# AntoinePassemiers/Oriana

Measured on NVIDIA B200. Metric: cavi_matrix_entries_per_sec, higher is better.
Workload: dtype tf32 operands / f32 accumulate (f32 state, f64 ELBO sums)

## Files before the change

include/oriana_b200.h:

```cpp
#ifndef ORIANA_B200_H
#define ORIANA_B200_H

#include <stddef.h>
#include <stdint.h>

#ifdef __cplusplus
extern "C" {
#endif

#define ORI_OK 0
#define ORI_EINVAL (-1)
#define ORI_ECUDA (-2)
#define ORI_ENODEV (-3)
#define ORI_EUNSUPPORTED (-4)

#define ORI_F_DROPOUT 1u
#define ORI_F_QUIRK 2u
#define ORI_F_ELBO 4u
#define ORI_F_NO_TENSOR 8u
#define ORI_F_SPARSE 16u
#define ORI_F_DEVICE_ITER 32u

#define ORI_F_PRECISE 64u
#define ORI_F_FIXED_CHAIN 128u
// ... 109 lines not shown
int ori_zigap_compute_Z_q_expectations_host(float* DZ_hat_i, float* DZ_hat_j, float* DZ_exp_logsum_hat,
                                            const float* log_U_hat, const float* log_V_hat,
                                            const float* D_hat, const float* X,
                                            int64_t n, int64_t p, int64_t K, int quirk);
int ori_gap_compute_Z_q_expectations_host(float* Z_hat_i, float* Z_hat_j,
                                          const float* log_U_hat, const float* log_V_hat,
                                          const float* X, int64_t n, int64_t p, int64_t K);
int ori_zigap_compute_Z_q_expectations_ctx(ori_ctx_t* ctx, float* DZ_hat_i, float* DZ_hat_j, float* DZ_exp_logsum_hat,
                                           const float* log_U_hat, const float* log_V_hat,
                                           const float* D_hat, const float* X,
                                           int64_t n, int64_t p, int64_t K, int quirk);
int ori_gap_compute_Z_q_expectations_ctx(ori_ctx_t* ctx, float* Z_hat_i, float* Z_hat_j,
                                         const float* log_U_hat, const float* log_V_hat,
                                         const float* X, int64_t n, int64_t p, int64_t K);

int ori_synth_counts_f32(float* X, int64_t ldx, int64_t row0, int64_t n_rows, int32_t p, int32_t K,
                         uint64_t seed, float zero_level, int nb, float* Ustar, float* Vstar, float* pi,
                         void* stream);

int ori_widen_counts_f32(const void* src, int elem_bytes, int64_t lds, float* dst, int64_t ldd,
                         int64_t rows, int32_t p, void* stream);

int ori_expand_bitmap_counts_f32(const uint32_t* bitmap, int64_t words_per_row, const uint8_t* nz,
                                 const int64_t* rowoff, int64_t base, float* dst, int64_t ldd, int64_t rows,
                                 int32_t p, void* stream);

int ori_scatter_counts_f32(float* X, int64_t ldx, int64_t row0, int64_t rows, int32_t p, const int32_t* row,
                           const int32_t* col, const float* val, int64_t count, void* stream);

#ifdef __cplusplus
// ... 4 lines not shown
```

oriana_b200/_lib.py:

```python
import ctypes as C
import os

_HERE = os.path.dirname(os.path.abspath(__file__))
LIB_PATH = os.environ.get('ORIANA_B200_LIB') or os.path.join(_HERE, 'lib', 'liboriana_b200.so')

ORI_F_DROPOUT, ORI_F_QUIRK, ORI_F_ELBO, ORI_F_NO_TENSOR, ORI_F_SPARSE, ORI_F_DEVICE_ITER, ORI_F_PRECISE = 1, 2, 4, 8, 16, 32, 64
ORI_F_FIXED_CHAIN = 128
ORI_F_DETERMINISTIC = 256
ORI_M_STEP, ORI_M_INIT, ORI_M_INIT_KEEP, ORI_M_FINALIZE, ORI_M_REFRESH = 0, 1, 2, 3, 4
R64_NSLOTS = 8
SCAL_SLOTS = 16

_fp = C.POINTER(C.c_float)
_dp = C.POINTER(C.c_double)


class OriProblem(C.Structure):
    _fields_ = [
        ('n_rows', C.c_int64), ('n_total', C.c_int64), ('ldx', C.c_int64),
        ('p', C.c_int32), ('K', C.c_int32), ('KP', C.c_int32), ('flags', C.c_uint32),
        ('iter', C.c_int32), ('trace_cap', C.c_int32),
        ('X', C.c_void_p),
        ('a1', C.c_void_p), ('a2', C.c_void_p),
        ('U_hat', C.c_void_p * 2), ('eU', C.c_void_p * 2),
# ... 37 lines not shown
    'ori_row_sums_f32': ([C.c_void_p, C.c_int64, C.c_int64, C.c_int32, C.c_void_p, C.c_void_p], C.c_int),
    'ori_column_sums_f64': ([C.c_void_p, C.c_int64, C.c_int64, C.c_int32, C.c_void_p, C.c_void_p], C.c_int),
    'ori_deviance_sums': ([_PP, C.c_int, C.c_void_p, C.c_void_p, C.c_void_p, C.c_void_p, C.c_void_p], C.c_int),
    'ori_zigap_compute_Z_q_expectations_host': ([C.c_void_p] * 7 + [C.c_int64] * 3 + [C.c_int], C.c_int),
    'ori_gap_compute_Z_q_expectations_host': ([C.c_void_p] * 5 + [C.c_int64] * 3, C.c_int),
    'ori_ctx_create': ([C.POINTER(C.c_void_p), C.c_int64], C.c_int),
    'ori_ctx_destroy': ([C.c_void_p], C.c_int),
    'ori_ctx_stats': ([C.c_void_p] + [C.POINTER(C.c_uint64)] * 4, C.c_int),
    'ori_zigap_compute_Z_q_expectations_ctx': ([C.c_void_p] * 8 + [C.c_int64] * 3 + [C.c_int], C.c_int),
    'ori_gap_compute_Z_q_expectations_ctx': ([C.c_void_p] * 6 + [C.c_int64] * 3, C.c_int),
    'ori_widen_counts_f32': ([C.c_void_p, C.c_int, C.c_int64, C.c_void_p, C.c_int64, C.c_int64, C.c_int32, C.c_void_p], C.c_int),
    'ori_expand_bitmap_counts_f32': ([C.c_void_p, C.c_int64, C.c_void_p, C.c_void_p, C.c_int64, C.c_void_p, C.c_int64, C.c_int64,
                                      C.c_int32, C.c_void_p], C.c_int),
    'ori_scatter_counts_f32': ([C.c_void_p, C.c_int64, C.c_int64, C.c_int64, C.c_int32, C.c_void_p, C.c_void_p, C.c_void_p,
                                C.c_int64, C.c_void_p], C.c_int),
    'ori_synth_counts_f32': ([C.c_void_p, C.c_int64, C.c_int64, C.c_int64, C.c_int32, C.c_int32, C.c_uint64,
                              C.c_float, C.c_int, C.c_void_p, C.c_void_p, C.c_void_p, C.c_void_p], C.c_int),
}

_lib = None


class OrianaB200Error(RuntimeError):
    pass


def exported_symbols():
    return sorted(_SIGNATURES)


# ... 39 lines not shown
```

oriana_b200/csrc/kernels_tc.cu:

```cuda
#include <cstring>
#include "common.cuh"
#include "tc_ptx.cuh"

namespace ori {
using namespace tc;

constexpr int TC_OWN = 128;
constexpr int NEW = 8;
constexpr int TC_THREADS = 64 + 32 * NEW;
constexpr int NCTA = 2;

template <int KP, bool PRECISE = false, bool DEVI = false>
struct Cfg {
    static_assert(KP == 32 || KP == 64, "tensor path: KP is 32 or 64");
    static_assert(!PRECISE || KP == 32, "the fp32-grade plan exists for KP = 32");
    static constexpr int SW = PRECISE ? 32 : 2048 / KP;
    static constexpr int NS = 2;
    static constexpr int KB = KP / 32;
    static constexpr int KST = 3, TST = 3, XST = 4;
    static constexpr int NTA = PRECISE ? 4 : 2;
    static constexpr uint32_t K_BLK = (SW / NCTA) * 128;
    static constexpr uint32_t K_ARR = KB * K_BLK;
    static constexpr uint32_t K_STAGE = 4 * K_ARR;
    static constexpr uint32_t T_CHUNK = (KP / NCTA) * 128;
// ... 55 lines not shown
    asm volatile("cp.async.bulk.shared::cluster.global.mbarrier::complete_tx::bytes [%0], [%1], %2, [%3];"
                 ::"r"(smem_u32(dst)), "l"(src), "r"(bytes), "r"(smem_u32(bar)) : "memory");
}
__device__ __forceinline__ uint32_t tf32_bias(float x) { return __float_as_uint(x) + 0x1000u; }

__device__ __forceinline__ float4 lds128(uint32_t a) {
    float4 v;
    asm volatile("ld.shared.v4.f32 {%0, %1, %2, %3}, [%4];" : "=f"(v.x), "=f"(v.y), "=f"(v.z), "=f"(v.w) : "r"(a));
    return v;
}
__device__ __forceinline__ float lds32(uint32_t a) {
    float v;
    asm volatile("ld.shared.f32 %0, [%1];" : "=f"(v) : "r"(a));
    return v;
}
__device__ __forceinline__ float sel_nz_a(float x, float a, float b) {
    float d;
    asm("{\n\t.reg .pred q;\n\tsetp.neu.f32 q, %1, 0f00000000;\n\tselp.f32 %0, %2, %3, q;\n\t}" : "=f"(d) : "f"(x), "f"(a), "f"(b));
    return d;
}
__device__ __forceinline__ float sel_nz_b(float x, float a, float b) {
    float d;
    asm("{\n\t.reg .pred q;\n\t.reg .f32 t;\n\tabs.f32 t, %1;\n\tsetp.gtu.f32 q, t, 0f00000000;\n\tselp.f32 %0, %2, %3, q;\n\t}"
        : "=f"(d) : "f"(x), "f"(a), "f"(b));
    return d;
}
__device__ __forceinline__ float is_zero_f(float x) {
    float d;
    asm("set.eq.f32.f32 %0, %1, 0f00000000;" : "=f"(d) : "f"(x));
    return d;
// ... 20 lines not shown
        }
    }
    __device__ __forceinline__ void init(const TcArgs& a, int ncta_, int rank_) {
        ncta = ncta_; rank = rank_;
        item = blockIdx.x / ncta; stride = gridDim.x / ncta;
        load(a);
    }
    __device__ __forceinline__ bool valid(const TcArgs& a) const { return item < a.n_items; }
    __device__ __forceinline__ bool first() const { return t == t_begin; }
    __device__ __forceinline__ bool last() const { return t == t_end - 1; }
    __device__ __forceinline__ void next(const TcArgs& a) {
        if (++t >= t_end) { item += stride; load(a); }
    }
};

template <bool GENES, bool DROPOUT, bool ELBO, int KP, bool PRECISE, bool DEVI = false, bool UFL = false, bool DET = false>
__global__ void __launch_bounds__(TC_THREADS, 1)
k_tc_pass(const __grid_constant__ TcMaps maps, const TcArgs a)
{
    using C = Cfg<KP, PRECISE, DEVI>;
    static_assert(!DEVI || (!GENES && DROPOUT && !ELBO && !PRECISE), "deviance pass: row orientation, two contractions");
    constexpr int SW = C::SW, NS = C::NS;
    constexpr uint32_t TM_UV = C::TM_UV;
    constexpr int KST = C::KST, TST = C::TST, XST = C::XST;
    constexpr uint32_t K_STAGE = C::K_STAGE, T_STAGE = C::T_STAGE, X_STAGE = C::X_STAGE, LP_STAGE = C::LP_STAGE;
    constexpr uint32_t OFF_K = C::OFF_K, OFF_T = C::OFF_T, OFF_X = C::OFF_X, OFF_LP = C::OFF_LP, OFF_BAR = C::OFF_BAR;
    constexpr uint32_t TM_STAGE = C::TM_STAGE, TM_ACC = C::TM_ACC, TM_A = C::TM_A, TM_COLS = C::TM_COLS;
    constexpr int B_KFULL = C::B_KFULL, B_KEMPTY = C::B_KEMPTY, B_TFULL = C::B_TFULL, B_TEMPTY = C::B_TEMPTY,
                  B_XFULL = C::B_XFULL, B_XEMPTY = C::B_XEMPTY, B_SREADY = C::B_SREADY, B_PREADY = C::B_PREADY,
                  B_ACC_READY = C::B_ACC_READY, B_ACC_FREE = C::B_ACC_FREE, B_A_READY = C::B_A_READY, NBARS = C::NBARS;
    constexpr int CW = SW / 2;
    constexpr int G = CW / 16;
    constexpr int NQ = DROPOUT ? 4 : 2;
    constexpr int NT = DROPOUT ? 2 : 1;
    const int rank = (int)cluster_ctarank();

// ... 65 lines not shown
                        for (int kb = 0; kb < C::KB; ++kb) {
                            uint8_t* dst = st + q * C::K_ARR + kb * C::K_BLK;
                            const int row = (int)(q * a.sw_pad + sw0 + (SW / NCTA) * rank);
                            tma_load_2d_pair(dst, &maps.swK, bar, 32 * kb, row, L2_EVICT_LAST);
                        }
                }
                __syncwarp();
            }
            {
                const uint32_t s = nk % XST;
                mbar_wait(&bars[B_XEMPTY + s], ((nk / XST) & 1) ^ 1, 11);
                if (elect_one()) {
                    uint8_t* st = smem + OFF_X + s * X_STAGE;
                    uint64_t* bar = &bars[B_XFULL + s];
                    const int sw0 = ik.t * SW;
                    mbar_expect_tx(bar, X_STAGE + ((!GENES && DROPOUT) ? LP_STAGE : 0));
                    if (DEVI) bulk_load(smem + OFF_LP + s * LP_STAGE, a.devlp + (long long)ik.t * (8 * SW), LP_STAGE, bar);
                    if (!GENES) {
#pragma unroll
                        for (int c = 0; c < SW / 32; ++c)
                            tma_load_2d_hint(st + c * (TC_OWN * 128), &maps.X, bar, sw0 + 32 * c, ik.own0, L2_EVICT_FIRST);
                        if (DROPOUT && !DEVI) {
                            bulk_load(smem + OFF_LP + s * LP_STAGE, a.lp2w + sw0, SW * 4, bar);
                            bulk_load(smem + OFF_LP + s * LP_STAGE + SW * 4, a.flw + sw0, SW * 4, bar);
                            bulk_load(smem + OFF_LP + s * LP_STAGE + SW * 8, a.cw + sw0, SW * 4, bar);
                        }
                    } else {
#pragma unroll
                        for (int c = 0; c < 4; ++c)
                            tma_load_2d_hint(st + c * (SW * 128), &maps.X, bar, ik.own0 + 32 * c, sw0, L2_EVICT_FIRST);
                    }
                }
                __syncwarp();
            }
            if (nk > 0) load_T();
            ++nk; ik.next(a);
        }
        if (nk > 0) load_T();
    } else if (warp == 1 || false) {
        if (rank == 0) {
            constexpr uint32_t idescS = make_idesc_tf32(TC_OWN * NCTA, SW, false, false);
// ... 130 lines not shown
                        plo[e] = pack_bf16x2(__uint_as_float(wlo[2 * e]), __uint_as_float(wlo[2 * e + 1]));
                    }
                    tmem_st8(tlane + TM_A + (2 * slice + 1) * KP + 8 * c16, phi);
                    tmem_st8(tlane + TM_A + (2 * slice + 1) * KP + KP / 2 + 8 * c16, plo);
                }
            }
            tmem_wait_st();
            tc_fence_before();
            __syncwarp();
            if (lane == 0) mbar_arrive_cluster(&bars[B_A_READY], 0);
        };

        uint32_t xoff[8];
#pragma unroll
        for (int k = 0; k < 8; ++k) xoff[k] = (uint32_t)(quarter * (SW * 128) + ((((lane >> 2) ^ k)) << 4) + (lane & 3) * 4);

        TileIter ti;
        ti.init(a, NCTA, rank);
        uint32_t it = 0;
        int li = 0;
        if (ti.valid(a)) a_load_store(ti.own0);
        while (ti.valid(a)) {
            const long long own_idx = (long long)ti.own0 + lrow;
            const bool own_ok = own_idx < a.own_total;
            const int next_item = ti.item + ti.stride;
            const bool has_next = next_item < a.n_items;
            const int next_own0 = ((next_item % a.n_own_units) * NCTA + rank) * TC_OWN;
            float lp2j = 0.f, flj = 0.f, cj = 0.f, ulim = 127.f;
            if (GENES && DROPOUT) {
                lp2j = a.lp2w[own_idx]; flj = a.flw[own_idx];
// ... 1 lines not shown
                ulim = fminf(127.f, 127.f + lp2j);
            }
            const float lp2f = fminf(lp2j, 3.0e38f);
            float thr_o = 0.f, den_lim = 0.f;
            if constexpr (UFL) {
                thr_o = own_ok ? a.thr_own[own_idx] : 0.f;
                den_lim = thr_o * __ldg(a.thr_sw_max);
                den_lim = den_lim == den_lim ? fminf(den_lim, 3.0e38f) : 0.f;
            }
            const bool slow_item = DROPOUT && (GENES ? (__any_sync(0xffffffffu, flj != 0.f || lp2j == -INFINITY) != 0) : any_floor);
            float cs = 0.f;
            float xl_s = 0.f, xl_c = 0.f, ent_s = 0.f, ent_c = 0.f;
            const int t_end = ti.t_end;
            uint32_t dr[2][16], ur[2][16];
            float x[2][16];
            struct Tile { uint32_t xs_addr, lp_addr, tden, s, xs; int valid; bool slow; long long sw0; };
            auto tile_of = [&](uint32_t it_, int t_) {
                Tile c;
                c.s = it_ % NS; c.xs = it_ % XST;
                c.xs_addr = sbase + OFF_X + c.xs * X_STAGE;
                c.lp_addr = sbase + OFF_LP + c.xs * LP_STAGE;
                c.valid = (int)min((long long)SW, a.sw_total - (long long)t_ * SW);
                c.sw0 = (long long)t_ * SW;
                c.slow = slow_item || (GENES && c.valid != SW);
                c.tden = tlane + c.s * TM_STAGE;
                return c;
            };
            auto wait_tile = [&](uint32_t it_) {
                const uint32_t s = it_ % NS, sph = (it_ / NS) & 1, xs = it_ % XST, xph = (it_ / XST) & 1;
                mbar_wait2(&bars[B_XFULL + xs], xph, &bars[B_SREADY + s], sph, 30);
// ... 12 lines not shown
                    w[e] = __float_as_uint(h0); w[e + 1] = __float_as_uint(h1);
                    ph[e >> 1] = pack_bf16x2(h0, h1);
                    pl[e >> 1] = pack_bf16x2(v0 - h0, v1 - h1);
                }
            };
            auto load_x = [&](const Tile& c, int g, int b) {
                const int c0 = colbase + g * 16;
                if (!GENES) {
                    const uint32_t base = c.xs_addr + (c0 >> 5) * (TC_OWN * 128) + lrow * 128;
                    const int cb = (c0 & 31) >> 2;
#pragma unroll
                    for (int q = 0; q < 4; ++q) {
                        const float4 v = lds128(base + (((cb + q) ^ (lrow & 7)) << 4));
                        x[b][4 * q] = v.x; x[b][4 * q + 1] = v.y; x[b][4 * q + 2] = v.z; x[b][4 * q + 3] = v.w;
                    }
                } else {
#pragma unroll
                    for (int e = 0; e < 16; ++e) {
                        const int i = c0 + e;
                        x[b][e] = lds32(c.xs_addr + xoff[i & 7] + i * 128);
                    }
                }
            };
            auto slow_group = [&](const Tile& c, int g, int b, float& t_xl, float& t_ent) {
                const int c0 = colbase + g * 16;
                tmem_ld16(c.tden + c0, dr[b]);
                if (DROPOUT) tmem_ld16(c.tden + TM_UV + c0, ur[b]);
                tmem_wait_ld();
#pragma unroll
                for (int e = 0; e < 16; ++e) {
                    const float den = __uint_as_float(dr[b][e]);
                    const float xe = x[b][e];
                    const bool nz = xe != 0.f;
                    float xr = xe;
                    if constexpr (UFL)
                        if (den_lim > 0.f && nz && (c0 + e) < c.valid && den < thr_o * __ldg(a.thr_sw + c.sw0 + c0 + e)) xr = 0.f;
                    const float dg = den > 0.f ? den : 1.f;
                    float tt = dg, e2 = 0.f, D = 1.f;
                    if (DROPOUT) {
                        const float lp2 = GENES ? lp2j : lds32(c.lp_addr + 4 * (c0 + e));
                        const float fl = GENES ? flj : lds32(c.lp_addr + SW * 4 + 4 * (c0 + e));
                        e2 = fminf(__uint_as_float(ur[b][e]) - lp2, 127.f);
                        tt = nz ? dg : 1.f + ex2_approx(e2);
                        const float r = rcp_approx(tt);
                        D = fmaxf(nz ? 1.f : r, fl);
                        dr[b][e] = PRECISE ? __float_as_uint(xr * r) : tf32_bias(xr * r);
                        ur[b][e] = PRECISE ? __float_as_uint(D) : tf32_bias(D);
// ... 13 lines not shown
            };
            auto fast_group = [&](const Tile& c, int g, int b, float& g_cs, float& g_xl, float& g_ent) -> float {
                const int c0 = colbase + g * 16;
                float cc[16];
                if (DROPOUT && !GENES) {
#pragma unroll
                    for (int q = 0; q < 4; ++q) {
                        const float4 v = lds128(c.lp_addr + SW * 8 + 4 * (c0 + 4 * q));
                        cc[4 * q] = v.x; cc[4 * q + 1] = v.y; cc[4 * q + 2] = v.z; cc[4 * q + 3] = v.w;
                    }
                }
                float dmin = 1.f;
#pragma unroll
                for (int e = 0; e < 16; ++e) {
                    const float den = __uint_as_float(dr[b][e]);
                    const float xe = x[b][e];
                    dmin = fminf(dmin, den);
                    float tt = den, uvp = 0.f;
                    if (DROPOUT) {
                        uvp = __uint_as_float(ur[b][e]);
                        if (GENES && ELBO) uvp = fminf(uvp, ulim);
                        const float tz = fmaf(ex2_approx(uvp), GENES ? cj : cc[e], 1.f);
                        tt = sel_nz_a(xe, den, tz);
                    }
                    const float r = rcp_approx(tt);
                    dr[b][e] = PRECISE ? __float_as_uint(xe * r) : tf32_bias(xe * r);
                    float D = 1.f;
                    if (DROPOUT) {
                        D = sel_nz_b(xe, 1.f, r);
                        ur[b][e] = PRECISE ? __float_as_uint(D) : tf32_bias(D);
                    }
// ... 477 lines not shown
                                            P->n_rows, w.np, P->KP);
    return check_launch("k_tc_prep(rows, logsum)");
}

static void tc_partition(TcArgs& a, bool genes, int units, int sw, bool precise, bool fixed_chain) {
    int tpc = (precise ? ORI_TC_CHUNK_PRECISE : (genes ? ORI_TC_CHUNK : 2 * ORI_TC_CHUNK)) / sw;
    if (tpc < 1) tpc = 1;
    if (tpc > a.n_sw_tiles) tpc = a.n_sw_tiles;
    const int min_tpc = (128 / sw) > 1 ? 128 / sw : 1;
    while (!fixed_chain && (long long)a.n_own_units * cdiv(a.n_sw_tiles, tpc) < units / 2 && tpc > min_tpc) tpc = (tpc + 1) / 2;
    a.tiles_per_chunk = tpc;
    a.n_chunks = cdiv(a.n_sw_tiles, a.tiles_per_chunk);
    a.n_items = a.n_own_units * a.n_chunks;
}

template <bool GENES, bool D, bool E, int KP, bool PRECISE, bool DEVI, bool UFL, bool DET>
static int launch_tc_variant(const TcMaps& maps, const TcArgs& a, int grid, cudaStream_t st) {
    auto kern = k_tc_pass<GENES, D, E, KP, PRECISE, DEVI, UFL, DET>;
    constexpr uint32_t smem = Cfg<KP, PRECISE, DEVI>::SMEM_BYTES;
    static bool attr_done = false;
    if (!attr_done) {
        cudaError_t e_ = cudaFuncSetAttribute(kern, cudaFuncAttributeMaxDynamicSharedMemorySize, smem);
        if (e_ != cudaSuccess) return set_error(ORI_ECUDA, "cudaFuncSetAttribute: %s", cudaGetErrorString(e_));
        attr_done = true;
    }
    cudaLaunchConfig_t cfg = {};
    cfg.gridDim = dim3(grid); cfg.blockDim = dim3(TC_THREADS); cfg.dynamicSmemBytes = smem; cfg.stream = st;
    cudaLaunchAttribute attr[1];
    attr[0].id = cudaLaunchAttributeClusterDimension;
    attr[0].val.clusterDim.x = NCTA; attr[0].val.clusterDim.y = 1; attr[0].val.clusterDim.z = 1;
    cfg.attrs = attr; cfg.numAttrs = 1;
    cudaError_t e_ = cudaLaunchKernelEx(&cfg, kern, maps, a);
    if (e_ != cudaSuccess) return set_error(ORI_ECUDA, "cudaLaunchKernelEx(k_tc_pass): %s", cudaGetErrorString(e_));
    return ORI_OK;
}

template <bool GENES, int KP, bool PRECISE, bool UFL, bool DET>
static int launch_tc_flags(bool drop, bool elbo, const TcMaps& maps, const TcArgs& a, int grid, cudaStream_t st) {
    if (drop && elbo) return launch_tc_variant<GENES, true, true, KP, PRECISE, false, UFL, DET>(maps, a, grid, st);
    if (drop) return launch_tc_variant<GENES, true, false, KP, PRECISE, false, UFL, DET>(maps, a, grid, st);
    if (elbo) return launch_tc_variant<GENES, false, true, KP, PRECISE, false, UFL, DET>(maps, a, grid, st);
    return launch_tc_variant<GENES, false, false, KP, PRECISE, false, UFL, DET>(maps, a, grid, st);
}

template <bool GENES, int KP, bool PRECISE>
static int launch_tc_pass_p(const ori_problem_t* P, int gen_old, cudaStream_t st, bool logsum = false) {
    using C = Cfg<KP, PRECISE>;
    const TcWs w = tc_carve(P);
    const bool sparse = P->flags & ORI_F_SPARSE;
    const bool drop = (P->flags & ORI_F_DROPOUT) && !logsum, elbo = (P->flags & ORI_F_ELBO) && !logsum;
    constexpr int SW = C::SW;
    TcMaps maps;
    TcArgs a;
    bool ok;
    if (!GENES) {
        ok = make_tmap_f32(&maps.swK, w.geneK, 4 * w.pp, KP, KP, 32, SW / NCTA) &&
             make_tmap_f32(&maps.swT, w.geneT, C::NTA * KP, w.pp, w.pp, 32, KP / NCTA) &&
             make_tmap_f32(&maps.X, P->X, P->n_rows, P->p, P->ldx, 32, TC_OWN);
        a.own_total = P->n_rows; a.sw_total = P->p; a.sw_pad = w.pp;
        a.own_e = P->eU[gen_old]; a.own_E = P->U_hat[gen_old];
        a.acc1 = P->Zi; a.acc2 = P->a2s;
    } else {
        ok = make_tmap_f32(&maps.swK, w.rowK, 4 * w.np, KP, KP, 32, SW / NCTA) &&
             make_tmap_f32(&maps.swT, w.rowT, C::NTA * KP, w.np, w.np, 32, KP / NCTA) &&
             make_tmap_f32(&maps.X, P->X, P->n_rows, P->p, P->ldx, 32, SW);
        a.own_total = P->p; a.sw_total = P->n_rows; a.sw_pad = w.np;
        a.own_e = sparse ? P->eVd : P->eV; a.own_E = sparse ? P->Vh_old : P->V_hat;
        a.acc1 = P->red32 + (logsum ? 2ll * P->p * KP : 0ll); a.acc2 = P->red32 + (long long)P->p * KP;
    }
    if (!ok) return set_error(ORI_ECUDA, "cuTensorMapEncodeTiled failed");
    a.lp2w = w.lp2w; a.flw = w.flw; a.cw = w.cw; a.any_floor = w.flags;
    const bool ufl = P->thrU && P->thrV;
    const float* thr_rows = ufl ? P->thrU + (long long)gen_old * P->n_rows : nullptr;
    a.thr_own = ufl ? (GENES ? P->thrV : thr_rows) : nullptr;
    a.thr_sw = ufl ? (GENES ? thr_rows : P->thrV) : nullptr;
    a.thr_sw_max = ufl ? reinterpret_cast<const float*>(w.flags + (GENES ? 2 : 1)) : nullptr;
    a.colsum = P->red64; a.part64 = P->red64 + P->p + 2 * P->KP;
    a.n_own_tiles = cdiv(a.own_total, TC_OWN);
    a.n_own_units = cdiv(a.n_own_tiles, NCTA);
    a.n_sw_tiles = cdiv(a.sw_total, SW);
// ... 8 lines not shown
        a.colsum2 = P->det_ws + (long long)DET_FU_BLOCKS * DET_FU_SLOTS;
        a.item_part = a.colsum2 + pad128(P->p);
        if (GENES && drop) {
            const cudaError_t e2 = cudaMemsetAsync(a.colsum2, 0, sizeof(double) * (size_t)P->p, st);
            if (e2 != cudaSuccess) return set_error(ORI_ECUDA, "cudaMemsetAsync(colsum2): %s", cudaGetErrorString(e2));
        }
        a.tickets = reinterpret_cast<int*>(a.item_part + det_max_items(P->n_rows, P->p) * DET_ITEM_SLOTS);
        cudaError_t e_ = cudaMemsetAsync(a.tickets, 0, sizeof(int) * (size_t)(a.n_own_tiles + 2), st);
        if (e_ != cudaSuccess) return set_error(ORI_ECUDA, "cudaMemsetAsync(tickets): %s", cudaGetErrorString(e_));
        if (!(GENES && elbo)) a.item_part = nullptr;
        else {
            e_ = cudaMemsetAsync(a.item_part, 0, sizeof(double) * (size_t)a.n_items * DET_ITEM_SLOTS, st);
            if (e_ != cudaSuccess) return set_error(ORI_ECUDA, "cudaMemsetAsync(item_part): %s", cudaGetErrorString(e_));
        }
    }
    const int rc = det ? launch_tc_flags<GENES, KP, PRECISE, false, true>(drop, elbo, maps, a, grid, st)
                 : ufl ? launch_tc_flags<GENES, KP, PRECISE, true, false>(drop, elbo, maps, a, grid, st)
                       : launch_tc_flags<GENES, KP, PRECISE, false, false>(drop, elbo, maps, a, grid, st);
    if (rc != ORI_OK) return rc;
    int extra = 0;
    if (det && GENES && drop) { k_det_add<<<cdiv(P->p, 256), 256, 0, st>>>(P->red64, a.colsum2, P->p); ++extra; }
    if (a.item_part) {
        double* part = P->red64 + P->p + 2 * P->KP;
        k_det_sum_items<<<1, 1024, 0, st>>>(a.item_part, (long long)a.n_items * (DET_ITEM_SLOTS / 2), part + R64_XLOGDEN, part + R64_ENT);
        ++extra;
    }
    if (extra) return check_launch("k_tc_pass + deterministic sums", 1 + extra);
    return check_launch(GENES ? "k_tc_pass(genes)" : "k_tc_pass(rows)");
}

template <bool GENES>
static int launch_tc_pass(const ori_problem_t* P, int gen_old, cudaStream_t st, bool logsum = false) {
    if (P->flags & ORI_F_PRECISE) return launch_tc_pass_p<GENES, 32, true>(P, gen_old, st, logsum);
// ... 37 lines not shown
    while ((long long)a.n_own_units * cdiv(a.n_sw_tiles, a.tiles_per_chunk) < 2LL * units && a.tiles_per_chunk > 4)
        a.tiles_per_chunk = (a.tiles_per_chunk + 1) / 2;
    a.n_chunks = cdiv(a.n_sw_tiles, a.tiles_per_chunk);
    a.n_items = a.n_own_units * a.n_chunks;
    const int grid = NCTA * (a.n_items < units ? a.n_items : units);
    const int rc = launch_tc_variant<false, true, false, KP, false, true, false, false>(maps, a, grid, st);
    if (rc != ORI_OK) return rc;
    return check_launch("k_tc_pass(deviance)");
}

int launch_deviance_tc(const ori_problem_t* P, int g, const double* pi, const double* cmean, long long* out_int, cudaStream_t st) {
    if (P->KP == 64) return launch_deviance_tc_kp<64>(P, g, pi, cmean, out_int, st);
    return launch_deviance_tc_kp<32>(P, g, pi, cmean, out_int, st);
}

int launch_pass_rows_tc(const ori_problem_t* P, int gen_old, cudaStream_t st) { return launch_tc_pass<false>(P, gen_old, st); }
int launch_pass_genes_tc(const ori_problem_t* P, int gen_old, cudaStream_t st) { return launch_tc_pass<true>(P, gen_old, st); }
int launch_pass_genes_logsum_tc(const ori_problem_t* P, int gen_old, cudaStream_t st) { return launch_tc_pass<true>(P, gen_old, st, true); }

}
```

oriana_b200/csrc/synth.cu:

```cuda
#include "common.cuh"

namespace ori {

struct Philox {
    uint32_t k0, k1;
    __device__ Philox(uint64_t seed) : k0((uint32_t)seed), k1((uint32_t)(seed >> 32)) {}
    __device__ uint4 operator()(uint32_t c0, uint32_t c1, uint32_t c2, uint32_t c3) const {
        uint32_t a = k0, b = k1;
#pragma unroll
        for (int r = 0; r < 10; ++r) {
            const uint32_t h0 = __umulhi(0xD2511F53u, c0), l0 = 0xD2511F53u * c0;
            const uint32_t h1 = __umulhi(0xCD9E8D57u, c2), l1 = 0xCD9E8D57u * c2;
            c0 = h1 ^ c1 ^ a; c1 = l1; c2 = h0 ^ c3 ^ b; c3 = l0;
            a += 0x9E3779B9u; b += 0xBB67AE85u;
        }
        return make_uint4(c0, c1, c2, c3);
    }
};

__device__ __forceinline__ float u01(uint32_t x) { return ((float)(x >> 8) + 0.5f) * (1.0f / 16777216.0f); }

__global__ void k_synth_factor(float* __restrict__ out, long long rows, int K, long long row0, uint64_t seed, uint32_t tag) {
    const long long idx = (long long)blockIdx.x * blockDim.x + threadIdx.x;
    if (idx >= rows * K) return;
// ... 180 lines not shown
    if (e >= count) return;
    const long long r = (long long)row[e] - row0;
    const int c = col[e];
    if (r >= 0 && r < rows && c >= 0 && c < p) X[r * ldx + c] = val[e];
}

extern "C" int ori_scatter_counts_f32(float* X, int64_t ldx, int64_t row0, int64_t rows, int32_t p, const int32_t* row,
                                      const int32_t* col, const float* val, int64_t count, void* stream)
{
    if (!X || ldx < p || p <= 0 || rows < 0 || count < 0 || (count && (!row || !col || !val)))
        return set_error(ORI_EINVAL, "ori_scatter_counts_f32: bad argument");
    if (count == 0 || rows == 0) return ORI_OK;
    k_scatter_counts<<<cdiv(count, 256), 256, 0, (cudaStream_t)stream>>>(X, ldx, row0, rows, p, row, col, val, count);
    return check_launch("k_scatter_counts");
}
```

oriana_b200/csrc/tc_ptx.cuh:

```cuda
#pragma once
#include <cuda.h>
#include <cuda_runtime.h>
#include <stdint.h>
#include <stdio.h>

namespace tc {

__device__ __forceinline__ uint32_t smem_u32(const void* p) { return (uint32_t)__cvta_generic_to_shared(p); }

__device__ __forceinline__ void mbar_init(uint64_t* bar, uint32_t count) {
    asm volatile("mbarrier.init.shared::cta.b64 [%0], %1;" ::"r"(smem_u32(bar)), "r"(count) : "memory");
}
__device__ __forceinline__ void fence_barrier_init() { asm volatile("fence.mbarrier_init.release.cluster;" ::: "memory"); }
__device__ __forceinline__ void mbar_expect_tx(uint64_t* bar, uint32_t bytes) {
    asm volatile("mbarrier.arrive.expect_tx.shared::cta.b64 _, [%0], %1;" ::"r"(smem_u32(bar)), "r"(bytes) : "memory");
}
__device__ __forceinline__ void mbar_arrive(uint64_t* bar) {
    asm volatile("mbarrier.arrive.shared::cta.b64 _, [%0];" ::"r"(smem_u32(bar)) : "memory");
}
__device__ __forceinline__ bool mbar_try_wait(uint64_t* bar, uint32_t parity) {
    uint32_t ok;
    asm volatile(
        "{\n\t.reg .pred p;\n\t"
        "mbarrier.try_wait.parity.shared::cta.b64 p, [%1], %2;\n\t"
// ... 206 lines not shown
}

inline bool make_tmap_f32(CUtensorMap* map, const float* base, uint64_t rows, uint64_t cols, uint64_t ld,
                          uint32_t box_cols, uint32_t box_rows) {
    EncodeTiledFn fn = get_encode_fn();
    if (!fn) return false;
    cuuint64_t dims[2] = {cols, rows};
    cuuint64_t strides[1] = {ld * sizeof(float)};
    cuuint32_t box[2] = {box_cols, box_rows};
    cuuint32_t estr[2] = {1, 1};
    return fn(map, CU_TENSOR_MAP_DATA_TYPE_FLOAT32, 2, (void*)base, dims, strides, box, estr,
              CU_TENSOR_MAP_INTERLEAVE_NONE, CU_TENSOR_MAP_SWIZZLE_128B, CU_TENSOR_MAP_L2_PROMOTION_L2_256B,
              CU_TENSOR_MAP_FLOAT_OOB_FILL_NONE) == CUDA_SUCCESS;
}

}
```

oriana_b200/models/base.py:

```python
from abc import ABCMeta, abstractmethod
import ctypes

import numpy as np
import torch

from .. import _lib
from ..dims import Dimensions
from ..nodes import Einsum
from ..parameters import Parameter
from ..problem import build_problem, gene_buffers, kernel_plan, row_pitch
from ..sharding import RowSharding
from ..singlecell.cmatrix import CountMatrix


class DeviceView(Parameter):

    def __init__(self, owner, getter, on_write=True):
        self._owner = owner
        self._getter = getter
        self._on_write = on_write

    @property
    def _t(self):
        return self._getter()

# ... 114 lines not shown
            return torch.zeros((p, KP), **f32)
        self._a1, self._a2, self._Zi = rowf(), rowf(), rowf()
        self._Uhat, self._eU = [rowf(), rowf()], [rowf(), rowf()]
        self._a2s = rowf() if self._dropout else None
        g = gene_buffers(p, K, KP, dev, dropout=self._dropout, sparse=self._sparse, trace_cap=self._trace_cap)
        self._b1, self._b2, self._Vhat, self._eV, self._red32 = g['b1'], g['b2'], g['V_hat'], g['eV'], g['red32']
        self._lp, self._pfloor, self._pi, self._hyper = g['lp'], g['pfloor'], g['pi_d'], g['hyper']
        self._red64, self._scal, self._trace = g['red64'], g['scal'], g['elbo_trace']
        self._xrow = xcol = None
        if self._flags & _lib.ORI_F_ELBO:
            self._xrow = torch.zeros((max(n, 1),), **f32)
            cs = torch.zeros((p,), **f64)
            _lib.check(self._lib.ori_row_sums_f32(self._X.data_ptr(), ldx, n, p, self._xrow.data_ptr(), _lib.stream_ptr()))
            _lib.check(self._lib.ori_column_sums_f64(self._X.data_ptr(), ldx, n, p, cs.data_ptr(), _lib.stream_ptr()))
            xcol = self._shard.allreduce_sum(cs).to(torch.float32)
        under = self.emulate_underflow
        self._arrays = dict(
            X=self._X, a1=self._a1, a2=self._a2, U_hat=self._Uhat, eU=self._eU, Zi=self._Zi, a2s=self._a2s,
            eUw=rowf() if (self._flags & _lib.ORI_F_QUIRK) else None, xrow=self._xrow, xcol=xcol,
            thrU=torch.zeros((2, max(n, 1)), **f32) if under else None, thrV=torch.zeros((p,), **f32) if under else None,
            tc_ws=torch.empty((int(self._lib.ori_tc_workspace_floats(n, p, KP)) + 32,), **f32) if self._tensor else None,
            det_ws=torch.zeros((int(self._lib.ori_det_workspace_doubles(n, p, KP)) + 8,), **f64) if self.deterministic else None,
            **g, **self._extra_fields(rowf, genef))
        P = self._P = build_problem(n_rows=n, n_total=self.n_total, ldx=ldx, p=p, K=K, KP=KP, flags=self._flags,
                                   trace_cap=self._trace_cap, **self._arrays)
        _lib.check(self._lib.ori_problem_check(ctypes.byref(P)))
        self.uses_tensor_path = bool(self._lib.ori_uses_tensor_path(ctypes.byref(P)))
        if self._tensor and not self.uses_tensor_path and n > 0:
            raise _lib.OrianaB200Error('tensor path requested but not available on this device / driver')

        K_ = K
        self.a1 = DeviceView(self, lambda: self._a1[:, :K_])
        self.a2 = DeviceView(self, lambda: self._a2[:, :K_])
        self.b1 = DeviceView(self, lambda: self._b1[:, :K_])
        self.b2 = DeviceView(self, lambda: self._b2[:, :K_])
        self.alpha1 = DeviceView(self, lambda: self._hyper[0])
        self.alpha2 = DeviceView(self, lambda: self._hyper[1])
        self.beta1 = DeviceView(self, lambda: self._hyper[2])
        self.beta2 = DeviceView(self, lambda: self._hyper[3])

    def _extra_fields(self, rowf, genef):
        return {}

    def _call(self, name, *args):
        self._P.iter = self._iter
        _lib.check(getattr(self._lib, name)(ctypes.byref(self._P), *args, _lib.stream_ptr()))

    def _nmf_warm_start(self):
        mode = self._nmf_mode
        if mode is None:
            mode = 'device' if (self._shard.enabled or self.n * self.p > 50_000_000) else 'host'
        if mode == 'host':
            if self._shard.enabled:
                raise ValueError("nmf='host' needs the whole matrix on one rank")
# ... 294 lines not shown
```

oriana_b200/problem.py:

```python
import ctypes

import torch

from . import _lib


def row_pitch(p):
    return (p + 3) // 4 * 4


def pad_k(K):
    for kp in (8, 16, 32, 64):
        if K <= kp:
            return kp
    raise ValueError('k=%d: the CUDA kernels support latent dimensions up to 64' % K)


def kernel_plan(k, entries, precise=False, tensor=None, force_simt=False, sparse=False):
    if sparse and k > 64:
        raise ValueError('SparseZIGaP supports k <= 64')
    if sparse and k > 32:
        if tensor:
            raise ValueError('SparseZIGaP: the tensor path needs k <= 32 (32 < k <= 64 runs on the CUDA-core kernels)')
        tensor = False
# ... 50 lines not shown
```

Baseline: 383.5 billion.

## Use a gene-major float16 copy of X for the tensor-core gene pass

At setup the model builds a transposed, gene-major float16 copy of the count matrix and registers it. When every count converts to float16 exactly, the gene pass loads X tiles through a 2D TMA map from that copy instead of four strided f32 loads, and widens the values in registers. This halves the X bytes streamed in the gene pass and replaces strided loads with one contiguous TMA tile. The cost is extra device memory, a one-time transpose kernel, and a global registry keyed by pointer that must be kept in sync with the matrix.

```diff
diff --git a/include/oriana_b200.h b/include/oriana_b200.h
--- a/include/oriana_b200.h
+++ b/include/oriana_b200.h
@@ -147,6 +147,12 @@
                                          const float* log_U_hat, const float* log_V_hat,
                                          const float* X, int64_t n, int64_t p, int64_t K);
 
+int ori_gene_major_x_f16(const float* X, int64_t ldx, int64_t n_rows, int32_t p, uint16_t* Xt, int64_t ldxt,
+                         int* inexact, void* stream);
+int ori_attach_gene_major_x(const float* X, int64_t ldx, int64_t n_rows, int32_t p, const uint16_t* Xt, int64_t ldxt);
+int ori_detach_gene_major_x(const float* X, const uint16_t* Xt);
+int ori_uses_gene_major_x(const ori_problem_t* P);
+
 int ori_synth_counts_f32(float* X, int64_t ldx, int64_t row0, int64_t n_rows, int32_t p, int32_t K,
                          uint64_t seed, float zero_level, int nb, float* Ustar, float* Vstar, float* pi,
                          void* stream);
diff --git a/oriana_b200/_lib.py b/oriana_b200/_lib.py
--- a/oriana_b200/_lib.py
+++ b/oriana_b200/_lib.py
@@ -75,6 +75,10 @@
                                       C.c_int32, C.c_void_p], C.c_int),
     'ori_scatter_counts_f32': ([C.c_void_p, C.c_int64, C.c_int64, C.c_int64, C.c_int32, C.c_void_p, C.c_void_p, C.c_void_p,
                                 C.c_int64, C.c_void_p], C.c_int),
+    'ori_gene_major_x_f16': ([C.c_void_p, C.c_int64, C.c_int64, C.c_int32, C.c_void_p, C.c_int64, C.c_void_p, C.c_void_p], C.c_int),
+    'ori_attach_gene_major_x': ([C.c_void_p, C.c_int64, C.c_int64, C.c_int32, C.c_void_p, C.c_int64], C.c_int),
+    'ori_detach_gene_major_x': ([C.c_void_p, C.c_void_p], C.c_int),
+    'ori_uses_gene_major_x': ([_PP], C.c_int),
     'ori_synth_counts_f32': ([C.c_void_p, C.c_int64, C.c_int64, C.c_int64, C.c_int32, C.c_int32, C.c_uint64,
                               C.c_float, C.c_int, C.c_void_p, C.c_void_p, C.c_void_p, C.c_void_p], C.c_int),
 }
diff --git a/oriana_b200/csrc/kernels_tc.cu b/oriana_b200/csrc/kernels_tc.cu
--- a/oriana_b200/csrc/kernels_tc.cu
+++ b/oriana_b200/csrc/kernels_tc.cu
@@ -1,4 +1,6 @@
 #include <cstring>
+#include <mutex>
+#include <vector>
 #include "common.cuh"
 #include "tc_ptx.cuh"
 
@@ -93,6 +95,16 @@
     asm volatile("ld.shared.f32 %0, [%1];" : "=f"(v) : "r"(a));
     return v;
 }
+__device__ __forceinline__ float f16lo_f32(uint32_t w) {
+    float v;
+    asm("{\n\t.reg .b16 l, h;\n\tmov.b32 {l, h}, %1;\n\tcvt.f32.f16 %0, l;\n\t}" : "=f"(v) : "r"(w));
+    return v;
+}
+__device__ __forceinline__ float f16hi_f32(uint32_t w) {
+    float v;
+    asm("{\n\t.reg .b16 l, h;\n\tmov.b32 {l, h}, %1;\n\tcvt.f32.f16 %0, h;\n\t}" : "=f"(v) : "r"(w));
+    return v;
+}
 __device__ __forceinline__ float sel_nz_a(float x, float a, float b) {
     float d;
     asm("{\n\t.reg .pred q;\n\tsetp.neu.f32 q, %1, 0f00000000;\n\tselp.f32 %0, %2, %3, q;\n\t}" : "=f"(d) : "f"(x), "f"(a), "f"(b));
@@ -143,12 +155,14 @@
     }
 };
 
-template <bool GENES, bool DROPOUT, bool ELBO, int KP, bool PRECISE, bool DEVI = false, bool UFL = false, bool DET = false>
+template <bool GENES, bool DROPOUT, bool ELBO, int KP, bool PRECISE, bool DEVI = false, bool UFL = false, bool DET = false,
+          bool XH = false>
 __global__ void __launch_bounds__(TC_THREADS, 1)
 k_tc_pass(const __grid_constant__ TcMaps maps, const TcArgs a)
 {
     using C = Cfg<KP, PRECISE, DEVI>;
     static_assert(!DEVI || (!GENES && DROPOUT && !ELBO && !PRECISE), "deviance pass: row orientation, two contractions");
+    static_assert(!XH || GENES, "the float16 copy of X is gene-major: gene pass only");
     constexpr int SW = C::SW, NS = C::NS;
     constexpr uint32_t TM_UV = C::TM_UV;
     constexpr int KST = C::KST, TST = C::TST, XST = C::XST;
@@ -244,7 +258,7 @@
                     uint8_t* st = smem + OFF_X + s * X_STAGE;
                     uint64_t* bar = &bars[B_XFULL + s];
                     const int sw0 = ik.t * SW;
-                    mbar_expect_tx(bar, X_STAGE + ((!GENES && DROPOUT) ? LP_STAGE : 0));
+                    mbar_expect_tx(bar, (XH ? X_STAGE / 2 : X_STAGE) + ((!GENES && DROPOUT) ? LP_STAGE : 0));
                     if (DEVI) bulk_load(smem + OFF_LP + s * LP_STAGE, a.devlp + (long long)ik.t * (8 * SW), LP_STAGE, bar);
                     if (!GENES) {
 #pragma unroll
@@ -255,6 +269,8 @@
                             bulk_load(smem + OFF_LP + s * LP_STAGE + SW * 4, a.flw + sw0, SW * 4, bar);
                             bulk_load(smem + OFF_LP + s * LP_STAGE + SW * 8, a.cw + sw0, SW * 4, bar);
                         }
+                    } else if (XH) {
+                        tma_load_2d_hint(st, &maps.X, bar, sw0, ik.own0, L2_EVICT_FIRST);
                     } else {
 #pragma unroll
                         for (int c = 0; c < 4; ++c)
@@ -415,6 +431,8 @@
         uint32_t xoff[8];
 #pragma unroll
         for (int k = 0; k < 8; ++k) xoff[k] = (uint32_t)(quarter * (SW * 128) + ((((lane >> 2) ^ k)) << 4) + (lane & 3) * 4);
+        const uint32_t xh_row = (uint32_t)lrow * (SW * 2);
+        const int xh_swz = SW == 64 ? (lrow & 7) : ((lrow >> 1) & 3);
 
         TileIter ti;
         ti.init(a, NCTA, rank);
@@ -446,6 +464,11 @@
             const int t_end = ti.t_end;
             uint32_t dr[2][16], ur[2][16];
             float x[2][16];
+            uint32_t xw[2][8];
+            auto x_of = [&](int b, int e) -> float {
+                if (XH) return (e & 1) ? f16hi_f32(xw[b][e >> 1]) : f16lo_f32(xw[b][e >> 1]);
+                return x[b][e];
+            };
             struct Tile { uint32_t xs_addr, lp_addr, tden, s, xs; int valid; bool slow; long long sw0; };
             auto tile_of = [&](uint32_t it_, int t_) {
                 Tile c;
@@ -488,6 +511,13 @@
                         const float4 v = lds128(base + (((cb + q) ^ (lrow & 7)) << 4));
                         x[b][4 * q] = v.x; x[b][4 * q + 1] = v.y; x[b][4 * q + 2] = v.z; x[b][4 * q + 3] = v.w;
                     }
+                } else if (XH) {
+#pragma unroll
+                    for (int h = 0; h < 2; ++h) {
+                        const float4 v = lds128(c.xs_addr + xh_row + ((((c0 >> 3) + h) ^ xh_swz) << 4));
+                        xw[b][4 * h] = __float_as_uint(v.x); xw[b][4 * h + 1] = __float_as_uint(v.y);
+                        xw[b][4 * h + 2] = __float_as_uint(v.z); xw[b][4 * h + 3] = __float_as_uint(v.w);
+                    }
                 } else {
 #pragma unroll
                     for (int e = 0; e < 16; ++e) {
@@ -504,7 +534,7 @@
 #pragma unroll
                 for (int e = 0; e < 16; ++e) {
                     const float den = __uint_as_float(dr[b][e]);
-                    const float xe = x[b][e];
+                    const float xe = x_of(b, e);
                     const bool nz = xe != 0.f;
                     float xr = xe;
                     if constexpr (UFL)
@@ -548,7 +578,7 @@
 #pragma unroll
                 for (int e = 0; e < 16; ++e) {
                     const float den = __uint_as_float(dr[b][e]);
-                    const float xe = x[b][e];
+                    const float xe = x_of(b, e);
                     dmin = fminf(dmin, den);
                     float tt = den, uvp = 0.f;
                     if (DROPOUT) {
@@ -1056,9 +1086,9 @@
     a.n_items = a.n_own_units * a.n_chunks;
 }
 
-template <bool GENES, bool D, bool E, int KP, bool PRECISE, bool DEVI, bool UFL, bool DET>
+template <bool GENES, bool D, bool E, int KP, bool PRECISE, bool DEVI, bool UFL, bool DET, bool XH = false>
 static int launch_tc_variant(const TcMaps& maps, const TcArgs& a, int grid, cudaStream_t st) {
-    auto kern = k_tc_pass<GENES, D, E, KP, PRECISE, DEVI, UFL, DET>;
+    auto kern = k_tc_pass<GENES, D, E, KP, PRECISE, DEVI, UFL, DET, XH>;
     constexpr uint32_t smem = Cfg<KP, PRECISE, DEVI>::SMEM_BYTES;
     static bool attr_done = false;
     if (!attr_done) {
@@ -1077,12 +1107,27 @@
     return ORI_OK;
 }
 
+template <bool GENES, int KP, bool PRECISE, bool UFL, bool DET, bool XH>
+static int launch_tc_flags(bool drop, bool elbo, const TcMaps& maps, const TcArgs& a, int grid, cudaStream_t st) {
+    if (drop && elbo) return launch_tc_variant<GENES, true, true, KP, PRECISE, false, UFL, DET, XH>(maps, a, grid, st);
+    if (drop) return launch_tc_variant<GENES, true, false, KP, PRECISE, false, UFL, DET, XH>(maps, a, grid, st);
+    if (elbo) return launch_tc_variant<GENES, false, true, KP, PRECISE, false, UFL, DET, XH>(maps, a, grid, st);
+    return launch_tc_variant<GENES, false, false, KP, PRECISE, false, UFL, DET, XH>(maps, a, grid, st);
+}
 template <bool GENES, int KP, bool PRECISE, bool UFL, bool DET>
-static int launch_tc_flags(bool drop, bool elbo, const TcMaps& maps, const TcArgs& a, int grid, cudaStream_t st) {
-    if (drop && elbo) return launch_tc_variant<GENES, true, true, KP, PRECISE, false, UFL, DET>(maps, a, grid, st);
-    if (drop) return launch_tc_variant<GENES, true, false, KP, PRECISE, false, UFL, DET>(maps, a, grid, st);
-    if (elbo) return launch_tc_variant<GENES, false, true, KP, PRECISE, false, UFL, DET>(maps, a, grid, st);
-    return launch_tc_variant<GENES, false, false, KP, PRECISE, false, UFL, DET>(maps, a, grid, st);
+static int launch_tc_x(bool drop, bool elbo, bool xh, const TcMaps& maps, const TcArgs& a, int grid, cudaStream_t st) {
+    if (GENES && xh) return launch_tc_flags<GENES, KP, PRECISE, UFL, DET, GENES>(drop, elbo, maps, a, grid, st);
+    return launch_tc_flags<GENES, KP, PRECISE, UFL, DET, false>(drop, elbo, maps, a, grid, st);
+}
+
+struct XtCopy { const float* X; long long ldx, n_rows; int p; const uint16_t* Xt; long long ldxt; };
+static std::mutex g_xt_mu;
+static std::vector<XtCopy> g_xt;
+static bool find_gene_major_x(const ori_problem_t* P, XtCopy* out) {
+    std::lock_guard<std::mutex> lk(g_xt_mu);
+    for (const XtCopy& c : g_xt)
+        if (c.X == P->X && c.ldx == P->ldx && c.p == P->p && P->n_rows <= c.n_rows) { *out = c; return true; }
+    return false;
 }
 
 template <bool GENES, int KP, bool PRECISE>
@@ -1095,6 +1140,8 @@
     TcMaps maps;
     TcArgs a;
     bool ok;
+    XtCopy xt;
+    const bool xh = GENES && find_gene_major_x(P, &xt);
     if (!GENES) {
         ok = make_tmap_f32(&maps.swK, w.geneK, 4 * w.pp, KP, KP, 32, SW / NCTA) &&
              make_tmap_f32(&maps.swT, w.geneT, C::NTA * KP, w.pp, w.pp, 32, KP / NCTA) &&
@@ -1105,7 +1152,8 @@
     } else {
         ok = make_tmap_f32(&maps.swK, w.rowK, 4 * w.np, KP, KP, 32, SW / NCTA) &&
              make_tmap_f32(&maps.swT, w.rowT, C::NTA * KP, w.np, w.np, 32, KP / NCTA) &&
-             make_tmap_f32(&maps.X, P->X, P->n_rows, P->p, P->ldx, 32, SW);
+             (xh ? make_tmap_f16(&maps.X, xt.Xt, P->p, P->n_rows, xt.ldxt, SW, TC_OWN)
+                    : make_tmap_f32(&maps.X, P->X, P->n_rows, P->p, P->ldx, 32, SW));
         a.own_total = P->p; a.sw_total = P->n_rows; a.sw_pad = w.np;
         a.own_e = sparse ? P->eVd : P->eV; a.own_E = sparse ? P->Vh_old : P->V_hat;
         a.acc1 = P->red32 + (logsum ? 2ll * P->p * KP : 0ll); a.acc2 = P->red32 + (long long)P->p * KP;
@@ -1144,9 +1192,9 @@
             if (e_ != cudaSuccess) return set_error(ORI_ECUDA, "cudaMemsetAsync(item_part): %s", cudaGetErrorString(e_));
         }
     }
-    const int rc = det ? launch_tc_flags<GENES, KP, PRECISE, false, true>(drop, elbo, maps, a, grid, st)
-                 : ufl ? launch_tc_flags<GENES, KP, PRECISE, true, false>(drop, elbo, maps, a, grid, st)
-                       : launch_tc_flags<GENES, KP, PRECISE, false, false>(drop, elbo, maps, a, grid, st);
+    const int rc = det ? launch_tc_x<GENES, KP, PRECISE, false, true>(drop, elbo, xh, maps, a, grid, st)
+                 : ufl ? launch_tc_x<GENES, KP, PRECISE, true, false>(drop, elbo, xh, maps, a, grid, st)
+                       : launch_tc_x<GENES, KP, PRECISE, false, false>(drop, elbo, xh, maps, a, grid, st);
     if (rc != ORI_OK) return rc;
     int extra = 0;
     if (det && GENES && drop) { k_det_add<<<cdiv(P->p, 256), 256, 0, st>>>(P->red64, a.colsum2, P->p); ++extra; }
@@ -1214,6 +1262,33 @@
     return launch_deviance_tc_kp<32>(P, g, pi, cmean, out_int, st);
 }
 
+}
+
+extern "C" int ori_attach_gene_major_x(const float* X, int64_t ldx, int64_t n_rows, int32_t p, const uint16_t* Xt, int64_t ldxt)
+{
+    if (!X || !Xt || p <= 0 || n_rows <= 0 || ldx < p || ldxt < n_rows || (ldxt & 7) || ((uintptr_t)Xt & 15))
+        return ori::set_error(ORI_EINVAL, "ori_attach_gene_major_x: bad argument");
+    std::lock_guard<std::mutex> lk(ori::g_xt_mu);
+    ori::g_xt.push_back(ori::XtCopy{X, ldx, n_rows, p, Xt, ldxt});
+    return ORI_OK;
+}
+
+extern "C" int ori_detach_gene_major_x(const float* X, const uint16_t* Xt)
+{
+    std::lock_guard<std::mutex> lk(ori::g_xt_mu);
+    for (size_t i = 0; i < ori::g_xt.size(); ++i)
+        if (ori::g_xt[i].X == X && ori::g_xt[i].Xt == Xt) { ori::g_xt.erase(ori::g_xt.begin() + i); return ORI_OK; }
+    return ori::set_error(ORI_EINVAL, "ori_detach_gene_major_x: no such copy attached");
+}
+
+extern "C" int ori_uses_gene_major_x(const ori_problem_t* P)
+{
+    ori::XtCopy c;
+    return (P && ori::tc_eligible(P) && ori::find_gene_major_x(P, &c)) ? 1 : 0;
+}
+
+namespace ori {
+
 int launch_pass_rows_tc(const ori_problem_t* P, int gen_old, cudaStream_t st) { return launch_tc_pass<false>(P, gen_old, st); }
 int launch_pass_genes_tc(const ori_problem_t* P, int gen_old, cudaStream_t st) { return launch_tc_pass<true>(P, gen_old, st); }
 int launch_pass_genes_logsum_tc(const ori_problem_t* P, int gen_old, cudaStream_t st) { return launch_tc_pass<true>(P, gen_old, st, true); }
diff --git a/oriana_b200/csrc/synth.cu b/oriana_b200/csrc/synth.cu
--- a/oriana_b200/csrc/synth.cu
+++ b/oriana_b200/csrc/synth.cu
@@ -1,3 +1,4 @@
+#include <cuda_fp16.h>
 #include "common.cuh"
 
 namespace ori {
@@ -218,3 +219,43 @@
     k_scatter_counts<<<cdiv(count, 256), 256, 0, (cudaStream_t)stream>>>(X, ldx, row0, rows, p, row, col, val, count);
     return check_launch("k_scatter_counts");
 }
+
+__global__ void __launch_bounds__(256)
+k_gene_major_f16(const float* __restrict__ X, long long ldx, long long n_rows, int p, __half* __restrict__ Xt,
+                 long long ldxt, int* __restrict__ inexact)
+{
+    __shared__ float tile[64][33];
+    const long long i0 = (long long)blockIdx.x * 64;
+    bool bad = false;
+    for (int j0 = blockIdx.y * 32; j0 < p; j0 += gridDim.y * 32) {
+        const int j = j0 + threadIdx.x;
+        for (int r = threadIdx.y; r < 64; r += 8) {
+            const long long i = i0 + r;
+            tile[r][threadIdx.x] = (i < n_rows && j < p) ? X[i * ldx + j] : 0.f;
+        }
+        __syncthreads();
+        const long long i = i0 + 2 * threadIdx.x;
+        for (int k = threadIdx.y; k < 32 && j0 + k < p; k += 8) {
+            if (i < ldxt) {
+                const float a = tile[2 * threadIdx.x][k], b = tile[2 * threadIdx.x + 1][k];
+                const __half2 h = __floats2half2_rn(a, b);
+                bad |= !(__low2float(h) == a && __high2float(h) == b);
+                *reinterpret_cast<__half2*>(Xt + (long long)(j0 + k) * ldxt + i) = h;
+            }
+        }
+        __syncthreads();
+    }
+    if (__any_sync(0xffffffffu, bad) && (threadIdx.x & 31) == 0) *inexact = 1;
+}
+
+extern "C" int ori_gene_major_x_f16(const float* X, int64_t ldx, int64_t n_rows, int32_t p, uint16_t* Xt, int64_t ldxt,
+                                    int* inexact, void* stream)
+{
+    if (!X || !Xt || !inexact || p <= 0 || n_rows < 0 || ldx < p || ldxt < n_rows || (ldxt & 7) || ((uintptr_t)Xt & 15))
+        return set_error(ORI_EINVAL, "ori_gene_major_x_f16: bad argument");
+    if (ldxt == 0) return ORI_OK;
+    const long long gy = cdiv(p, 32);
+    const dim3 grid((unsigned)cdiv(ldxt, 64), (unsigned)(gy < 65535 ? gy : 65535));
+    k_gene_major_f16<<<grid, dim3(32, 8), 0, (cudaStream_t)stream>>>(X, ldx, n_rows, p, reinterpret_cast<__half*>(Xt), ldxt, inexact);
+    return check_launch("k_gene_major_f16");
+}
diff --git a/oriana_b200/csrc/tc_ptx.cuh b/oriana_b200/csrc/tc_ptx.cuh
--- a/oriana_b200/csrc/tc_ptx.cuh
+++ b/oriana_b200/csrc/tc_ptx.cuh
@@ -244,4 +244,17 @@
               CU_TENSOR_MAP_FLOAT_OOB_FILL_NONE) == CUDA_SUCCESS;
 }
 
-}
+inline bool make_tmap_f16(CUtensorMap* map, const void* base, uint64_t rows, uint64_t cols, uint64_t ld,
+                          uint32_t box_cols, uint32_t box_rows) {
+    EncodeTiledFn fn = get_encode_fn();
+    if (!fn || (box_cols != 64 && box_cols != 32)) return false;
+    cuuint64_t dims[2] = {cols, rows};
+    cuuint64_t strides[1] = {ld * 2};
+    cuuint32_t box[2] = {box_cols, box_rows};
+    cuuint32_t estr[2] = {1, 1};
+    return fn(map, CU_TENSOR_MAP_DATA_TYPE_FLOAT16, 2, (void*)base, dims, strides, box, estr,
+              CU_TENSOR_MAP_INTERLEAVE_NONE, box_cols == 64 ? CU_TENSOR_MAP_SWIZZLE_128B : CU_TENSOR_MAP_SWIZZLE_64B,
+              CU_TENSOR_MAP_L2_PROMOTION_L2_256B, CU_TENSOR_MAP_FLOAT_OOB_FILL_NONE) == CUDA_SUCCESS;
+}
+
+}
diff --git a/oriana_b200/models/base.py b/oriana_b200/models/base.py
--- a/oriana_b200/models/base.py
+++ b/oriana_b200/models/base.py
@@ -1,5 +1,6 @@
 from abc import ABCMeta, abstractmethod
 import ctypes
+import weakref
 
 import numpy as np
 import torch
@@ -8,7 +9,7 @@
 from ..dims import Dimensions
 from ..nodes import Einsum
 from ..parameters import Parameter
-from ..problem import build_problem, gene_buffers, kernel_plan, row_pitch
+from ..problem import build_problem, gene_buffers, gene_major_pitch, kernel_plan, row_pitch
 from ..sharding import RowSharding
 from ..singlecell.cmatrix import CountMatrix
 
@@ -153,6 +154,7 @@
             _lib.check(self._lib.ori_row_sums_f32(self._X.data_ptr(), ldx, n, p, self._xrow.data_ptr(), _lib.stream_ptr()))
             _lib.check(self._lib.ori_column_sums_f64(self._X.data_ptr(), ldx, n, p, cs.data_ptr(), _lib.stream_ptr()))
             xcol = self._shard.allreduce_sum(cs).to(torch.float32)
+        self._Xt = self._gene_major_x(ldx) if (self._tensor and n > 0) else None
         under = self.emulate_underflow
         self._arrays = dict(
             X=self._X, a1=self._a1, a2=self._a2, U_hat=self._Uhat, eU=self._eU, Zi=self._Zi, a2s=self._a2s,
@@ -167,6 +169,10 @@
         self.uses_tensor_path = bool(self._lib.ori_uses_tensor_path(ctypes.byref(P)))
         if self._tensor and not self.uses_tensor_path and n > 0:
             raise _lib.OrianaB200Error('tensor path requested but not available on this device / driver')
+        self._Xt_detach = None
+        if self._Xt is not None:
+            _lib.check(self._lib.ori_attach_gene_major_x(self._X.data_ptr(), ldx, n, p, self._Xt.data_ptr(), gene_major_pitch(n)))
+            self._Xt_detach = weakref.finalize(self, self._lib.ori_detach_gene_major_x, self._X.data_ptr(), self._Xt.data_ptr())
 
         K_ = K
         self.a1 = DeviceView(self, lambda: self._a1[:, :K_])
@@ -177,6 +183,28 @@
         self.alpha2 = DeviceView(self, lambda: self._hyper[1])
         self.beta1 = DeviceView(self, lambda: self._hyper[2])
         self.beta2 = DeviceView(self, lambda: self._hyper[3])
+
+    def _gene_major_x(self, ldx):
+        ldxt = gene_major_pitch(self.n)
+        try:
+            Xt = torch.empty((self.p, ldxt), dtype=torch.float16, device=self._dev)
+        except torch.cuda.OutOfMemoryError:
+            return None
+        inexact = torch.zeros((1,), dtype=torch.int32, device=self._dev)
+        _lib.check(self._lib.ori_gene_major_x_f16(self._X.data_ptr(), ldx, self.n, self.p, Xt.data_ptr(), ldxt,
+                                                  inexact.data_ptr(), _lib.stream_ptr()))
+        return None if int(inexact.item()) else Xt
+
+    def _drop_gene_major_x(self):
+        if self._Xt_detach is not None:
+            self._Xt_detach()
+            self._Xt = self._Xt_detach = None
+            if self._graphs:
+                self._graphs.clear()
+
+    @property
+    def gene_major_x(self):
+        return bool(self._lib.ori_uses_gene_major_x(ctypes.byref(self._P)))
 
     def _extra_fields(self, rowf, genef):
         return {}
diff --git a/oriana_b200/problem.py b/oriana_b200/problem.py
--- a/oriana_b200/problem.py
+++ b/oriana_b200/problem.py
@@ -7,6 +7,10 @@
 
 def row_pitch(p):
     return (p + 3) // 4 * 4
+
+
+def gene_major_pitch(n):
+    return (n + 7) // 8 * 8
 
 
 def pad_k(K):
```

Measured after the change: 414.0 billion, median of 6. 7.9% higher.
